# sashajenner/honours

Measured on AMD Instinct MI355X. Metric: raw-signal MB/s (compress+decompress), higher is better.
Workload: dtype u16

## Files before the change

honours_amd/csrc/press_abi.hip:

```cpp

#include <dlfcn.h>
#include <stdarg.h>
#include <stdio.h>
#include <stdlib.h>
#include <string.h>

#include <mutex>
#include <thread>
#include <algorithm>
#include <vector>

#include "../../include/press_hip.h"
#include "press_internal.h"
#include "zs_table.h"

using namespace ph;


static thread_local char g_err[256] = "";

static int fail(int code, const char *fmt, ...)
{
	va_list ap;
	va_start(ap, fmt);
// ... 13 lines not shown

int ph::set_error(int code, const char *fmt, ...)
{
	va_list ap;
	va_start(ap, fmt);
	vsnprintf(g_err, sizeof g_err, fmt, ap);
	va_end(ap);
	return code;
}


namespace {

struct DevBuf;
DevBuf *g_bufs = nullptr;

struct DevBuf {
	void *p = nullptr;
	size_t cap = 0;
	DevBuf *next;
	DevBuf() : next(g_bufs) { g_bufs = this; }
	DevBuf(const DevBuf &) = delete;
	DevBuf &operator=(const DevBuf &) = delete;
	int reserve(size_t n)
	{
		if (n <= cap)
			return 0;
		if (p)
			(void) hipFree(p);
		p = nullptr;
		cap = 0;
		size_t want = n + n / 8 + 4096;
		hipError_t e = hipMalloc(&p, want);
		if (e != hipSuccess)
			return fail(PRESS_HIP_EHIP, "hipMalloc(%zu): %s", want, hipGetErrorString(e));
		cap = want;
		return 0;
	}
	void release()
	{
		if (p)
			(void) hipFree(p);
		p = nullptr;
		cap = 0;
	}
};

struct Ctx {
	bool ready = false;
	int device = -1;
	hipStream_t own = nullptr;
	hipStream_t user = nullptr;
	bool use_user = false;
	DevBuf meta, ex_pos, ex_val, low, huff, chunks, gran, ctl, first_chunk, htiles, hunit, hrec, hlist, hread, hwave, hbits, hend, hmin, cbits;
	DevBuf ztmp, zoff, zoff4, zlen, zhist, ztab, zfirst, zblk, zsbits, zbpos, zbflag, zkcnt, zrd, znb, zn, zdcopy, zdhuf, zdunit, zdtree, zdlong, zdctl, zdseq, zdxblk;
	DevBuf sig, off, nsamp, arena, arena_off, lens, lens2, outn, dense, dense_off;
	uint64_t zs_total = 0;
	uint32_t zs_nhost = 0;
	uint32_t *zs_pin = nullptr;
	hipEvent_t zs_ev = nullptr;
	bool have_table = false;
	bool table_trie = false;
	uint32_t tlen[256];
	uint64_t tbits[256];

	hipStream_t stream() const { return use_user ? user : own; }
};

Ctx g;
std::recursive_mutex g_mu;
#define API_LOCK std::lock_guard<std::recursive_mutex> api_lock_(g_mu)
void staging_release();

int ctx_init()
{
	if (g.ready) {
		HIPCHK(hipSetDevice(g.device));
		return 0;
	}
	int ndev = 0;
	hipError_t e = hipGetDeviceCount(&ndev);
	if (e != hipSuccess || ndev == 0)
		return fail(PRESS_HIP_EHIP, "no HIP device: %s", hipGetErrorString(e));
	if (g.device < 0)
		HIPCHK(hipGetDevice(&g.device));
	HIPCHK(hipSetDevice(g.device));
	HIPCHK(hipStreamCreateWithFlags(&g.own, hipStreamNonBlocking));
	g.ready = true;
	return 0;
}

struct Zstd {
	bool tried = false;
	size_t (*compress)(void *, size_t, const void *, size_t, int) = nullptr;
	size_t (*decompress)(void *, size_t, const void *, size_t) = nullptr;
	size_t (*bound)(size_t) = nullptr;
	unsigned (*is_error)(size_t) = nullptr;
} zstd_fn;

bool zstd_open()
{
	if (zstd_fn.tried)
		return zstd_fn.compress != nullptr;
	zstd_fn.tried = true;
	struct { const char *name; int flags; } names[] = {
		{ "libzstd.so.1", RTLD_NOW | RTLD_LOCAL | RTLD_NOLOAD },
		{ "libzstd.so.1", RTLD_NOW | RTLD_LOCAL },
// ... 296 lines not shown
{
	if (g.meta.reserve(((size_t) nreads + 1) * sizeof(ReadMeta)))
		return PRESS_HIP_EHIP;
	if (is_zs(method)) {
		const int rc = reserve_scratch(zs_inner(method), total_samples, nreads, decode);
		if (rc)
			return rc;
	}
	if (is_zs(method) && decode) {
		ZsBufs z;
		zs_bufs(z, total_samples, nreads, method);
		const size_t nr = (size_t) nreads + 1;
		if (g.ztmp.reserve(2 * zs_tmp_bytes(method, total_samples, nreads)) || g.zoff.reserve(nr * 8) || g.zoff4.reserve(nr * 8) ||
		    g.zlen.reserve(nr * 8) || g.zrd.reserve(nr * sizeof(ZsRead)) || g.zn.reserve(nr * 4) ||
		    g.zdseq.reserve((size_t) z.cap_seq * sizeof(ZsSeq)) || g.zdxblk.reserve((size_t) z.cap_xblk * sizeof(ZsXBlk)) ||
		    g.zdcopy.reserve((size_t) z.cap_copy * sizeof(ZsCopy)) || g.zdhuf.reserve((size_t) z.cap_units * 8 * sizeof(ZsHuf)) ||
		    g.zdunit.reserve((size_t) z.cap_units * sizeof(ZsUnit)) || g.zdtree.reserve((size_t) z.cap_trees * sizeof(ZsTree)) || g.zdlong.reserve((size_t) z.cap_long * sizeof(ZsLong)) ||
		    g.zdctl.reserve(sizeof(ZsDCtl)))
			return PRESS_HIP_EHIP;
	}
	if (is_zs(method) && !decode) {
		const size_t mc = max_chunks_of(total_samples, nreads), mb = max_zblocks_of(total_samples, nreads);
		const size_t nr = (size_t) nreads + 1;
		if (g.ztmp.reserve(zs_tmp_bytes(method, total_samples, nreads)) || g.zoff.reserve(nr * 8) || g.zoff4.reserve(nr * 8) ||
		    g.zlen.reserve(nr * 8) || g.zhist.reserve(nr * 1024) || g.ztab.reserve(nr * sizeof(zs::Table)) ||
		    g.zfirst.reserve(nr * 4) || g.zblk.reserve(mb * 4) || g.zsbits.reserve(mb * 16) || g.zbpos.reserve(mb * 4) ||
		    g.zbflag.reserve(mb) || g.zkcnt.reserve(mc * 4) ||
		    g.zrd.reserve(nr * sizeof(ZsRead)) || g.znb.reserve(64) ||
		    g.ex_pos.reserve((total_samples + 64) * 4) || g.ex_val.reserve((total_samples + 64) * 4))
			return PRESS_HIP_EHIP;
	}
	if (is_svb(method) || is_ex(method)) {
		const size_t mc = max_chunks_of(total_samples, nreads);
		if (g.chunks.reserve(mc * sizeof(ChunkDesc)) || g.gran.reserve(2 * mc * sizeof(uint64_t)) ||
		    g.ctl.reserve(2 * sizeof(ChunkCtl)) || g.first_chunk.reserve(((size_t) nreads + 1) * 4))
			return PRESS_HIP_EHIP;
	}
	if (is_ex(method)) {
		if (g.ex_pos.reserve((total_samples + 64) * 4) || g.ex_val.reserve((total_samples + 64) * 4))
			return PRESS_HIP_EHIP;
		if (!decode && is_shuff(method)) {
			const size_t mc = max_chunks_of(total_samples, nreads);
			if (g.cbits.reserve(mc * sizeof(ChunkBits)))
				return PRESS_HIP_EHIP;
		}
		if (is_rc(method) && g.low.reserve(total_samples + 64))
			return PRESS_HIP_EHIP;
		if (decode && is_shuff(method)) {
			const size_t mt = max_htiles_of(total_samples, nreads);
			if (g.low.reserve(total_samples + 64) || g.htiles.reserve(mt * sizeof(HufTile)) ||
			    g.hunit.reserve(mt * (HUF_HT / 64) * sizeof(HufUnit)) || g.hrec.reserve(mt * HUF_HT * 4) ||
			    g.hlist.reserve(hlist_cap_of(mt) * 8) || g.hread.reserve(((size_t) nreads + 1) * 8) ||
			    g.hwave.reserve(mt * (HUF_HT / 64) * 8) || g.hbits.reserve(mt * (HUF_HT / 64) * 8) ||
			    g.hend.reserve(mt * HUF_HT + 64) ||
			    g.hmin.reserve(((size_t) nreads + 1) * 4))
				return PRESS_HIP_EHIP;
		}
	}
	return 0;
}

}


namespace {
constexpr int KT_RING = 128;
struct KTime {
	bool on = false;
	hipEvent_t ev[2][KT_RING][2];
	bool made = false;
	int n[2] = { 0, 0 };
} kt;
}

namespace ph {
static bool kt_muted = false;
void ktime_mute(bool m) { kt_muted = m; }
void ktime_begin(int which, hipStream_t s)
{
	if (kt.on && !kt_muted && kt.n[which] < KT_RING)
		(void) hipEventRecord(kt.ev[which][kt.n[which]][0], s);
}
void ktime_end(int which, hipStream_t s)
{
	if (kt.on && !kt_muted && kt.n[which] < KT_RING) {
		(void) hipEventRecord(kt.ev[which][kt.n[which]][1], s);
		kt.n[which]++;
	}
}
}

extern "C" int press_hip_kernel_timing(int enable)
{
	API_LOCK;
	int rc = ctx_init();
	if (rc)
		return rc;
	if (enable && !kt.made) {
		for (int w = 0; w < 2; w++)
			for (int i = 0; i < KT_RING; i++)
				for (int e = 0; e < 2; e++)
					HIPCHK(hipEventCreate(&kt.ev[w][i][e]));
		kt.made = true;
	}
	kt.on = enable != 0;
	kt.n[0] = kt.n[1] = 0;
	return 0;
// ... 677 lines not shown
		return rc;
	launch_symbol_counts((const int16_t *) g.sig.p, (const uint64_t *) g.off.p, (const uint32_t *) g.nsamp.p, nreads,
			     (uint64_t *) g.lens.p, g.chunks.p, nchunks, mc, (uint32_t) std::min<uint64_t>(grid, nch), s);
	hipError_t e = hipGetLastError();
	if (e != hipSuccess)
		return fail(PRESS_HIP_EHIP, "kernel launch: %s", hipGetErrorString(e));
	HIPCHK(hipMemcpyAsync(counts, g.lens.p, 257 * 8, hipMemcpyDeviceToHost, s));
	HIPCHK(hipStreamSynchronize(s));
	return 0;
}

extern "C" int press_hip_depress_batch(int method, const uint8_t *in, const uint64_t *in_off,
				       const uint64_t *in_len, uint32_t nreads, int16_t *sig,
				       const uint64_t *off, const uint32_t *n, uint64_t total_samples,
				       uint32_t *out_n, int device_resident)
{
	API_LOCK;
	int rc = ctx_init();
	if (rc)
		return rc;
	if ((rc = check_method(method)))
		return rc;
	if (nreads == 0)
		return 0;
	if (!in || !in_off || !in_len || !sig || !off || !n || !out_n)
		return fail(PRESS_HIP_EARG, "NULL argument");
	hipStream_t s = g.stream();
	if ((rc = reserve_scratch(method, total_samples, nreads, true)))
		return rc;
	g.zs_total = total_samples;

	DecodeArgs a;
	memset(&a, 0, sizeof a);
	a.nreads = nreads;
	a.meta = (ReadMeta *) g.meta.p;
	a.ex_pos = (uint32_t *) g.ex_pos.p;
	a.ex_val = (uint32_t *) g.ex_val.p;
	a.low = (uint8_t *) g.low.p;
	a.huff = (const HuffDev *) g.huff.p;
	a.chunks = (ChunkDesc *) g.chunks.p;
	a.gran = (uint64_t *) g.gran.p;
	a.ctl = (ChunkCtl *) g.ctl.p;
	a.first_chunk = (uint32_t *) g.first_chunk.p;
	a.max_chunks = max_chunks_of(total_samples, nreads);
	if (is_shuff(method)) {
		a.htiles = (HufTile *) g.htiles.p;
		a.hunit = (HufUnit *) g.hunit.p;
		a.hrec = (uint32_t *) g.hrec.p;
		a.hlist = (uint32_t *) g.hlist.p;
		a.hread = (uint32_t *) g.hread.p;
		a.hwave = (uint2 *) g.hwave.p;
		a.hbits = (unsigned long long *) g.hbits.p;
		a.hend = (uint8_t *) g.hend.p;
		a.hmin = (uint32_t *) g.hmin.p;
		a.max_htiles = max_htiles_of(total_samples, nreads);
		a.hlist_cap = (uint32_t) hlist_cap_of(a.max_htiles);
		a.huf_minlen = table_minlen() | (g.table_trie ? HUF_NEEDS_TRIE : 0u);
	}

	if (device_resident) {
		if ((uintptr_t) sig & 15)
			return fail(PRESS_HIP_EARG, "sig must be 16-byte aligned");
		a.in = in;
		a.in_off = in_off;
		a.in_len = in_len;
		a.sig = sig;
		a.off = off;
		a.nsamp = n;
		a.out_n = out_n;
		return launch_depress(method, a, s);
	}

	uint64_t dense = 0;
	std::vector<uint64_t> doff(nreads);
	std::vector<Piece> pc;
	pc.reserve(nreads);
	for (uint32_t r = 0; r < nreads; r++) {
		if (off[r] & 7)
			return fail(PRESS_HIP_EARG, "off[%u] is not a multiple of 8 samples", r);
		if (off[r] + n[r] > total_samples)
			return fail(PRESS_HIP_EARG, "slot %u ends beyond total_samples", r);
		doff[r] = dense;
		if (in_len[r])
			pc.push_back({ const_cast<uint8_t *>(in) + in_off[r], dense, in_len[r] });
		dense += in_len[r];
	}
	if (g.sig.reserve(total_samples * 2 + 64) || g.off.reserve((size_t) nreads * 8) ||
	    g.nsamp.reserve((size_t) nreads * 4) || g.arena.reserve(dense + 64) || g.arena_off.reserve((size_t) nreads * 8) ||
	    g.lens2.reserve((size_t) nreads * 8) || g.outn.reserve((size_t) nreads * 4))
		return PRESS_HIP_EHIP;
	HIPCHK(hipMemcpyAsync(g.arena_off.p, doff.data(), (size_t) nreads * 8, hipMemcpyHostToDevice, s));
	HIPCHK(hipMemcpyAsync(g.lens2.p, in_len, (size_t) nreads * 8, hipMemcpyHostToDevice, s));
	HIPCHK(hipMemcpyAsync(g.off.p, off, (size_t) nreads * 8, hipMemcpyHostToDevice, s));
	HIPCHK(hipMemcpyAsync(g.nsamp.p, n, (size_t) nreads * 4, hipMemcpyHostToDevice, s));
	if (nreads <= 4) {
		for (const Piece &q : pc)
			HIPCHK(hipMemcpyAsync((uint8_t *) g.arena.p + q.dense, q.host, q.len, hipMemcpyHostToDevice, s));
	} else if ((rc = staged_pieces<true>((uint8_t *) g.arena.p, dense, pc, s))) {
		return rc;
	}
	a.in = (const uint8_t *) g.arena.p;
	a.in_off = (const uint64_t *) g.arena_off.p;
	a.in_len = (const uint64_t *) g.lens2.p;
	a.sig = (int16_t *) g.sig.p;
	a.off = (const uint64_t *) g.off.p;
	a.nsamp = (const uint32_t *) g.nsamp.p;
// ... 576 lines not shown
```

honours_amd/csrc/press_huffman.hip:

```cpp

#include "press_internal.h"
#include "press_packed.h"
#include <cstddef>
#include <type_traits>

namespace ph {

#ifdef HUF_STAMPS
__device__ unsigned long long g_hstamp[32];
#define HSTAMP_DECL                                             \
	unsigned long long hs_t = __builtin_amdgcn_s_memtime(); \
	unsigned long long hs_acc[8] = { 0, 0, 0, 0, 0, 0, 0, 0 }
#define HSTAMP(i)                                                              \
	do {     \
		__builtin_amdgcn_sched_barrier(0);                             \
		const unsigned long long hs_n = __builtin_amdgcn_s_memtime(); \
		hs_acc[(i) & 7] += hs_n - hs_t;                                \
		hs_t = hs_n;                                                   \
		__builtin_amdgcn_sched_barrier(0);                             \
	} while (0)
#define HSTAMP_FLUSH(base)                                                     \
	do {                                                                   \
		if ((threadIdx.x & 63) == 0)                                   \
			for (int hs_i = 0; hs_i < 8; hs_i++)                   \
// ... 85 lines not shown
#pragma unroll
		for (int j = 0; j < NDW / 4; j++)
			t[j] = ld16_pay(q + 16 * j);
#pragma unroll
		for (int j = 0; j < NDW % 4; j++)
			x[j] = ld4_pay(q + 4 * (NDW / 4 * 4 + j));
#pragma unroll
		for (int j = 0; j < NDW / 4; j++) {
			col[(4 * j + 0) * S] = t[j].x;
			col[(4 * j + 1) * S] = t[j].y;
			col[(4 * j + 2) * S] = t[j].z;
			col[(4 * j + 3) * S] = t[j].w;
		}
#pragma unroll
		for (int j = 0; j < NDW % 4; j++)
			col[(NDW / 4 * 4 + j) * S] = x[j];
	} else if (nby > lo) {
		uint8_t b[4 * NDW];
#pragma unroll
		for (int i = 0; i < 4 * NDW; i++) {
			const int32_t r = rb0 + i;
			b[i] = src[r < lo ? lo : (r >= nby ? nby - 1 : r)];
		}
#pragma unroll
		for (int j = 0; j < NDW; j++) {
			uint32_t x = 0;
#pragma unroll
			for (int i = 0; i < 4; i++) {
				const int32_t r = rb0 + 4 * j + i;
				x |= (r >= lo && r < nby) ? (uint32_t) b[4 * j + i] << (8 * i) : 0u;
			}
			col[j * S] = x;
		}
	} else {
#pragma unroll
		for (int j = 0; j < NDW; j++)
			col[j * S] = 0;
	}
}

__device__ __forceinline__ int32_t unzz8(uint32_t z) { return (int32_t) (z >> 1) ^ -(int32_t) (z & 1u); }

typedef __attribute__((address_space(3))) const uint32_t *lds_cu32p;
typedef __attribute__((address_space(3))) const uint16_t *lds_cu16p;
typedef __attribute__((address_space(3))) const uint8_t *lds_cu8p;
typedef __attribute__((address_space(3))) uint8_t *lds_u8p;

struct LenTabs {
	alignas(16) uint32_t alut[1 << HUF_LUT_BITS];
	alignas(16) uint16_t flut[1 << HUF_LUT_BITS];
	alignas(16) uint16_t l2ld[HUF_L2_ENTRIES];
};

template <bool TRIE, int S = 64>
__device__ __forceinline__ uint32_t len_scan(const uint32_t *col_, const LenTabs *tabs, const HuffDev *hd, uint32_t start,
					     uint32_t lim, uint32_t nb, uint32_t &cnt, uint32_t &dsum)
{
	const lds_cu32p col = (lds_cu32p) col_;
	const lds_cu32p alut = (lds_cu32p) tabs->alut;
	const lds_cu16p flut = (lds_cu16p) tabs->flut;
	const lds_cu16p l2ld = (lds_cu16p) tabs->l2ld;
	bool bad = start == HEND;
	uint32_t L = lim < nb ? lim : nb;
	if (bad)
		L = 0;
	auto long_ld = [&](uint32_t e, uint32_t wnd) -> uint32_t {
		if (TRIE && e == 0xFFFFFFFFu) {
			const uint32_t t = trie_code(hd, wnd);
			return t ? (((t >> 24) & 31u) | (((uint32_t) unzz8(t & 0xFFu) & 0xFFu) << 8)) : 0u;
		}
		const uint32_t v = l2ld[(e & 0xFFFu) + ((wnd >> HUF_LUT_BITS) & ((1u << ((e >> 12) & 15u)) - 1u))];
		return v == 0xFFFFu ? 0u : v;
	};
	constexpr uint32_t PB = 30;
	const lds_cu32p colm = col - S;
	uint32_t A = (bad ? 0u : start) + PB;
	{
		int32_t LmP = (int32_t) L - HUF_LUT_BITS + (int32_t) PB;
		uint32_t jj = (A >> 5) & 15u;
		uint32_t w0 = colm[__umul24(jj, (uint32_t) S)], w1 = colm[__umul24(jj, (uint32_t) S) + S];
		while ((int32_t) (A & 0x1FFu) <= LmP) {
			const uint32_t pp = A & 0x1FFu;
			{
				const uint32_t w2 = colm[__umul24(jj, (uint32_t) S) + 2 * S];
				const uint32_t wnd = __builtin_amdgcn_alignbit(w1, w0, A);
				const uint32_t e = *(lds_cu32p) ((lds_cu8p) alut + (wnd & (((1u << HUF_LUT_BITS) - 1u) << 2)));
				uint32_t inc = e;
				if ((int32_t) e < 0) {
					const uint32_t ld = long_ld(e, wnd >> 2);
					const uint32_t tot = ld & 0xFFu;
					inc = tot | (1u << HUF_A_CNT) | (((uint32_t) (int32_t) (int8_t) (ld >> 8) & 0x7FFFu) << HUF_A_SUM);
					if (tot - 1u >= L + PB - pp) {
						inc = 0;
						LmP = -1;
					}
				}
				A += inc;
				const uint32_t jn = (A >> 5) & 15u;
				if (jn != jj) {
					w0 = w1;
					w1 = w2;
				}
				jj = jn;
			}
		}
	}
	uint32_t p = (A & 0x1FFu) - PB;
	uint32_t c = (A >> HUF_A_CNT) & 0x7Fu;
	int32_t d = (int32_t) (A << 1) >> 17;
	for (;;) {
		const bool act = p < L;
		if (!any64(act))
			break;
		const uint32_t pp = act ? p : 0u;
		const uint32_t j = pp >> 5;
		const int r0 = (int) __umul24(j, (uint32_t) S);
		const uint32_t wnd = __builtin_amdgcn_alignbit(col[r0 + S], col[r0], pp);
		const uint32_t e = alut[wnd & ((1u << HUF_LUT_BITS) - 1u)];
		const uint32_t f = flut[wnd & ((1u << HUF_LUT_BITS) - 1u)];
		uint32_t tot = e & 15u, n = (e >> HUF_A_CNT) & 15u, len1 = f & 0xFFu;
		int32_t dall = (int32_t) (e << 1) >> 17, d1 = (int32_t) (int8_t) (f >> 8);
		bool fail = false;
		if (any64(act && (int32_t) e < 0)) {
			if (act && (int32_t) e < 0) {
				const uint32_t ld = long_ld(e, wnd);
				tot = len1 = ld & 0xFFu;
				dall = d1 = (int32_t) (int8_t) (ld >> 8);
				fail = tot == 0;
				n = 1;
			}
		}
		const bool fits = pp + tot <= L;
		const bool cut = !fits && pp + len1 > nb;
		if (act && !fail && !cut) {
			p += fits ? tot : len1;
			c += fits ? n : 1u;
			d += fits ? dall : d1;
		}
		if (act && (fail || cut)) {
			bad = true;
			L = 0;
		}
	}
	cnt = c;
	dsum = (uint32_t) d & 0xFFFFu;
	return bad ? HEND : (p >= nb && p < lim ? HEND : p);
}

__device__ __forceinline__ void wave_lds_sync()
{
	__builtin_amdgcn_fence(__ATOMIC_RELEASE, "wavefront");
	__builtin_amdgcn_wave_barrier();
	__builtin_amdgcn_fence(__ATOMIC_ACQUIRE, "wavefront");
}



#ifndef HUF_SYNC_PER_CU
#define HUF_SYNC_PER_CU 2
// ... 69 lines not shown
	__syncthreads();
	uint32_t *img = imgs[threadIdx.x >> 6];
	for (uint32_t i = lane; i < 2 * S; i += 64)
		img[NDW * S + i] = 0;
	uint32_t *col = img + lane;
	HSTAMP_DECL;
	for (;;) {
		uint32_t u = 0;
		if (lane == 0) {
			const uint32_t t = atomicAdd(&s_ticket, 1u);
			const uint32_t c = t / SYNC_UC, slot = t % SYNC_UC;
			unsigned long long *cs = &s_chunk[c & 63u];
			if (slot == 0) {
				u = atomicAdd(&a.ctl->sunits, SYNC_UC);
				__hip_atomic_store(cs, ((unsigned long long) c << 32) | u, __ATOMIC_RELAXED, __HIP_MEMORY_SCOPE_WORKGROUP);
			} else {
				unsigned long long v;
				do {
					v = __hip_atomic_load(cs, __ATOMIC_RELAXED, __HIP_MEMORY_SCOPE_WORKGROUP);
				} while ((uint32_t) (v >> 32) != c);
				u = (uint32_t) v + slot;
			}
		}
		u = uniform(u);
		if (u >= nunits)
			break;
		HSTAMP(0);
		const uint32_t k = u / (HT / 64);
		const uint32_t tid = (u % (HT / 64)) * 64 + lane;
		const HufTile *dp = a.htiles + k;
		const uint32_t nbits_t = uniform(dp->nbits);
		const uint32_t t = uniform(dp->t_last) & 0x7FFFFFFFu;
		const uint8_t *src = a.in + dp->src;
		const int32_t nby = (int32_t) ((nbits_t + 7) >> 3);
		const bool exact = t == 0 && tid < 64;

		wave_lds_sync();
		col_load<NDW, S>(col, src, (int32_t) tid * (OWN / 8), 0, nby);
		wave_lds_sync();
		HSTAMP(1);
		const uint32_t nb = clamp_nb((int64_t) nbits_t - (int64_t) tid * OWN);

		uint32_t f, c0, c, dz, dv;
		{
			const uint32_t g = len_scan<TRIE, S>(col, &lds.tabs, a.huff, (uint32_t) (OWN - RUNUP), OWN, nb, c0, dz);
			const uint32_t gl = (uint32_t) __shfl_up((int) g, 1, 64);
			f = gl == HEND ? HEND : gl - OWN;
			if (gl == HEND && nb > 0)
				f = 0;
			if (lane == 0)
				f = nb > 0 ? 0u : HEND;
		}
		HSTAMP(2);
		const uint32_t e = len_scan<TRIE, S>(col, &lds.tabs, a.huff, f, OWN, nb, c, dv);
		HSTAMP(3);
		const uint32_t e8 = e == HEND ? R_END : e - OWN;
		const uint32_t cw = wave_scan(c), dw = wave_scan(dv);
		const uint32_t f8 = f == HEND ? R_END : f;
		const uint32_t pe8 = (uint32_t) __shfl_up((int) e8, 1, 64);
		const bool broken = lane ? f8 != pe8 : !exact;
		const unsigned long long bm = __ballot(broken);
		a.hrec[(uint64_t) k * HT + tid] = pack_rec(f, c, dv);
		a.hend[(uint64_t) k * HT + tid] = (uint8_t) e8;
		if (lane == 63) {
			a.hwave[u] = make_uint2(cw, dw & 0xFFFFu);
			a.hbits[u] = bm;
		}
		HSTAMP(4);
	}
	HSTAMP_FLUSH(0);
}

constexpr int LIST_WG = 1024;
__global__ __launch_bounds__(LIST_WG) void k_huf_list(DecodeArgs a)
{
	__shared__ uint32_t s_w[LIST_WG / 64];
	__shared__ uint32_t s_base;
	const uint32_t n = min(uniform(a.ctl->nchunks), a.max_htiles) * (HT / 64);
	const uint32_t u = blockIdx.x * LIST_WG + threadIdx.x;
	const uint32_t lane = threadIdx.x & 63, w = threadIdx.x >> 6;
	unsigned long long bm = u < n ? a.hbits[u] : 0ull;
	const uint32_t cnt = (uint32_t) __popcll(bm);
	const uint32_t inc = wave_scan(cnt);
	if (lane == 63)
		s_w[w] = inc;
	__syncthreads();
	uint32_t before = 0, total = 0;
#pragma unroll
	for (int i = 0; i < LIST_WG / 64; i++) {
		const uint32_t x = s_w[i];
		if (i < (int) w)
			before += x;
		total += x;
	}
	if (threadIdx.x == 0)
		s_base = total ? atomicAdd(&a.ctl->ticket2, total) : 0u;
	__syncthreads();
	uint32_t at = s_base + before + inc - cnt;
	while (bm) {
		const uint32_t b = (uint32_t) __builtin_ctzll(bm);
		bm &= bm - 1;
		if (at < a.hlist_cap)
			a.hlist[at] = u * 64 + b;
		at++;
	}
}

#ifndef HUF_FIX_WG
#define HUF_FIX_WG 1024
#endif
constexpr int FIX_WG = HUF_FIX_WG;
template <int RU, bool TRIE>
__global__ __launch_bounds__(FIX_WG) void k_huf_fix(DecodeArgs a, int round, int last)
{
	constexpr int OWN = HufGeo<RU>::OWN, NDW = HufGeo<RU>::NDW, NCOL = HufGeo<RU>::NCOL;
	struct Lds {
		LenTabs tabs;
		uint32_t imgs[FIX_WG / 64][NCOL * 64 + 64];
	};
	__shared__ __attribute__((aligned(16))) Lds lds;
	auto &imgs = lds.imgs;

	const uint32_t *in_list = a.hlist + (round & 1 ? a.hlist_cap : 0u);
	uint32_t *out_list = a.hlist + (round & 1 ? 0u : a.hlist_cap);
	const uint32_t *in_cnt = round ? &a.ctl->lists[round - 1] : &a.ctl->ticket2;
	uint32_t *out_cnt = &a.ctl->lists[round];
	const uint32_t n = min(uniform(*in_cnt), a.hlist_cap);
	if ((uint32_t) FIX_WG * blockIdx.x >= n)
		return;
	const uint32_t lane = threadIdx.x & 63;
	load_len_tables(a.huff, &lds.tabs, FIX_WG);
	__syncthreads();
	uint32_t *col = imgs[threadIdx.x >> 6] + lane;
	for (uint32_t i0 = FIX_WG * blockIdx.x + (threadIdx.x & ~63u); i0 < n; i0 += (uint32_t) FIX_WG * gridDim.x) {
		uint32_t ent = i0 + lane < n ? in_list[i0 + lane] : LIST_NONE;
		if (ent != LIST_NONE && (a.hrec[ent] & 0xFFu) == a.hend[ent - 1])
			ent = LIST_NONE;
		const bool mine = ent != LIST_NONE;
		const uint64_t g = mine ? ent : 1u;
		const uint32_t k = (uint32_t) (g / HT), tid = (uint32_t) (g % HT);
		const HufTile *dp = a.htiles + k;
		const uint32_t nbits_t = mine ? dp->nbits : 0u;
		wave_lds_sync();
		if (mine)
			col_load<NDW>(col, a.in + dp->src, (int32_t) tid * (OWN / 8), 0, (int32_t) ((nbits_t + 7) >> 3));
		wave_lds_sync();
		const uint32_t pe = mine ? a.hend[g - 1] : R_END;
		const uint32_t old_e = mine ? a.hend[g] : R_END;
		uint32_t c2, d2;
		const uint32_t e2 = len_scan<TRIE>(col, &lds.tabs, a.huff, (!mine || pe == R_END) ? HEND : pe, OWN,
					     clamp_nb((int64_t) nbits_t - (int64_t) tid * OWN), c2, d2);
		const uint32_t e8 = e2 == HEND ? R_END : e2 - OWN;
		bool next = false;
		if (mine) {
			const uint32_t old = a.hrec[g];
			a.hrec[g] = pack_rec(pe == R_END ? HEND : pe, c2, d2);
			const long long dc = (long long) (int32_t) (c2 - ((old >> 8) & 0xFFu));
			const unsigned long long dd = (d2 - (old >> 16)) & 0xFFFFu;
			if (dc != 0 || dd != 0)
				atomicAdd(reinterpret_cast<unsigned long long *>(a.hwave + (uint64_t) k * (HT / 64) + (tid >> 6)),
					  (dd << 32) + (unsigned long long) dc);
			if (e8 != old_e) {
				a.hend[g] = (uint8_t) e8;
				const bool more = tid + 1 < HT || !(dp->t_last >> 31);
				next = more && (uint64_t) tid * OWN + OWN < nbits_t;
			}
		}
		list_push(out_list, out_cnt, a.hlist_cap, next, (uint32_t) g + 1, lane);
		if (last && next)
			atomicMin(&a.hmin[dp->read], (uint32_t) g + 1);
	}
}

template <int RU, bool TRIE>
__global__ __launch_bounds__(64) void k_huf_serial(DecodeArgs a)
{
	constexpr int OWN = HufGeo<RU>::OWN, NDW = HufGeo<RU>::NDW, NCOL = HufGeo<RU>::NCOL;
	struct Lds {
		LenTabs tabs;
		uint32_t img[NCOL * 64 + 64];
	};
	__shared__ __attribute__((aligned(16))) Lds lds;
	auto &img = lds.img;

	const uint32_t r = blockIdx.x;
	const uint32_t g0 = uniform(a.hmin[r]);
	if (g0 == 0xFFFFFFFFu)
		return;
	const uint32_t lane = threadIdx.x;
	const uint32_t k0 = uniform(a.hread[2 * r]), nt = uniform(a.hread[2 * r + 1]);
	load_len_tables(a.huff, &lds.tabs, 64);
	uint32_t *col = img + lane;
	const uint64_t gend = (uint64_t) (k0 + nt) * HT;
	for (uint64_t g = g0; g < gend; g++) {
		const uint32_t k = (uint32_t) (g / HT), tid = (uint32_t) (g % HT);
		const HufTile *dp = a.htiles + k;
		const uint32_t nbits_t = uniform(dp->nbits);
		if ((uint64_t) tid * OWN >= nbits_t)
			break;
		const uint32_t pe = uniform((uint32_t) __hip_atomic_load(a.hend + g - 1, __ATOMIC_RELAXED, __HIP_MEMORY_SCOPE_AGENT));
		const uint32_t rec = uniform(__hip_atomic_load(a.hrec + g, __ATOMIC_RELAXED, __HIP_MEMORY_SCOPE_AGENT));
		if ((rec & 0xFFu) == pe)
			continue;
		wave_lds_sync();
		if (lane == 0)
			col_load<NDW>(col, a.in + dp->src, (int32_t) tid * (OWN / 8), 0, (int32_t) ((nbits_t + 7) >> 3));
		wave_lds_sync();
		uint32_t c2, d2;
		const uint32_t e2 = len_scan<TRIE>(col, &lds.tabs, a.huff, (lane || pe == R_END) ? HEND : pe, OWN,
					     clamp_nb((int64_t) nbits_t - (int64_t) tid * OWN), c2, d2);
		if (lane == 0) {
			a.hrec[g] = pack_rec(pe == R_END ? HEND : pe, c2, d2);
			atomicAdd(reinterpret_cast<unsigned long long *>(a.hwave + (uint64_t) k * (HT / 64) + (tid >> 6)),
				  ((unsigned long long) ((d2 - (rec >> 16)) & 0xFFFFu) << 32) +
					  (unsigned long long) (long long) (int32_t) (c2 - ((rec >> 8) & 0xFFu)));
			__hip_atomic_store(a.hend + g, (uint8_t) (e2 == HEND ? R_END : e2 - OWN), __ATOMIC_RELAXED, __HIP_MEMORY_SCOPE_AGENT);
		}
		__builtin_amdgcn_fence(__ATOMIC_RELEASE, "agent");
	}
}

__device__ __forceinline__ uint32_t unzz16(uint32_t z) { return ((z >> 1) ^ (0u - (z & 1u))) & 0xFFFFu; }

__device__ __forceinline__ void keys_below2(const uint32_t *pos, uint32_t nex, uint32_t ka, uint32_t kb, uint32_t &ea, uint32_t &eb)
{
	uint32_t la = 0, lb = 0;
	for (uint32_t step = nex ? 1u << (31 - __builtin_clz(nex)) : 0u; step; step >>= 1) {
		const uint32_t ia = la + step - 1, ib = lb + step - 1;
		const uint32_t pa = ia < nex ? pos[ia] : 0u, pb = ib < nex ? pos[ib] : 0u;
		if (ia < nex && pa - ia < ka)
			la += step;
		if (ib < nex && pb - ib < kb)
			lb += step;
	}
	ea = la;
	eb = lb;
}

template <int RU>
__global__ __launch_bounds__(HT) void k_huf_chain(DecodeArgs a)
{
	constexpr uint32_t UB = 64 * HufGeo<RU>::OWN / 8;
	constexpr uint32_t UPT = HT / 64;
	__shared__ uint32_t s_w[HT / 64], s_wd[HT / 64];
	__shared__ unsigned long long s_cum;

	const uint32_t r = blockIdx.x;
	const uint32_t tid = threadIdx.x;
	const uint32_t k0 = uniform(a.hread[2 * r]), nt = uniform(a.hread[2 * r + 1]);
	if (!nt)
		return;
	const uint32_t nu = nt * UPT;
	const uint2 *hw = a.hwave + (uint64_t) k0 * UPT;
	if (tid == 0)
		s_cum = 0;
	__syncthreads();
	{
		uint64_t c = 0;
		for (uint32_t u = tid; u < nu; u += HT)
			c += hw[u].x;
		if (c)
			atomicAdd(&s_cum, (unsigned long long) c);
	}
	const uint32_t want = uniform(a.htiles[k0].want);
	const uint32_t nex = uniform(a.meta[r].nex);
// ... 50 lines not shown
#pragma unroll
		for (int w2 = 0; w2 < HT / 64; w2++) {
			const uint32_t x = s_w[w2], y = s_wd[w2];
			if (w2 < (int) (tid >> 6)) {
				before += x;
				dbefore += y;
			}
			total += x;
			dtotal += y;
		}
		if (u < nu) {
			const uint64_t ob = cum + before + inc - c;
			const uint32_t L0 = ob > 0xFFFFFFFFull ? 0xFFFFFFFFu : (uint32_t) ob;
			const uint32_t quota = L0 >= want ? 0u : (c < want - L0 ? c : want - L0);
			const uint32_t L1 = L0 + quota;
			uint32_t Ea = 0, Eb = 0;
			if (fused && quota) {
				keys_below2(pos, nex, L0, L1, Ea, Eb);
				if (L1 == nlow)
					Eb = nex;
			}
			uint32_t bz = zd0;
			if (L0) {
				bz = unzz16(zd0) + ((dcum + dbefore + dinc - dt) & 0xFFFFu);
				if (Ea) {
					const uint32_t pv = val[Ea - 1];
					bz += (pv >> 16) + unzz16(pv & 0xFFFFu);
				}
				bz &= 0xFFFFu;
			}
			const uint64_t src = src0 + (uint64_t) u * UB;
			const int64_t nby = nby0 - (int64_t) u * UB;
			const uint32_t nbyc = nby <= 0 ? 0u : (nby > (int64_t) HUF_U_NBY ? HUF_U_NBY : (uint32_t) nby);
			uint4 *d = reinterpret_cast<uint4 *>(a.hunit + (uint64_t) k0 * UPT + u);
			d[0] = make_uint4((uint32_t) src, (uint32_t) (src >> 32) | (bz << 16), (uint32_t) o0, (uint32_t) (o0 >> 32));
			d[1] = make_uint4(L0, quota | (nbyc << 14) | ((q & 15u) << 26) | (fused ? 1u << 30 : 0u), Ea, Eb - Ea);
		}
		cum += total;
		dcum += dtotal;
		__syncthreads();
	}
	static_assert(HUF_U_QUOTA >= 64u * 255u, "a unit's quota");
	if (tid == 0) {
		a.meta[r].nlow = nlow;
		if (fused)
			a.hread[2 * r + 1] = nt | HUF_FUSED;
	}
}


constexpr uint32_t EMIT_STG = 4096;

template <bool TRIE>
__device__ __forceinline__ void emit_codes(const uint32_t *col_, const uint32_t *lut_, const uint16_t *lut2_,
					   const HuffDev *hd, uint32_t p, uint32_t nmine, uint8_t *wp_)
{
	const lds_cu32p col = (lds_cu32p) col_;
	const lds_cu8p lut = (lds_cu8p) lut_;
	const lds_cu16p lut2 = (lds_cu16p) lut2_;
	auto long_entry = [&](uint32_t e, uint32_t wnd) -> uint32_t {
		if (TRIE && e == 0xFFFFFFFFu) {
			const uint32_t t = trie_code(hd, wnd);
			return t ? ((t & 0xFFFFFF00u) | ((uint32_t) unzz8(t & 0xFFu) & 0xFFu)) : 0u;
		}
		const uint32_t e2 = lut2[(e & 0xFFFu) + ((wnd >> HUF_LUT_BITS) & ((1u << ((e >> 12) & 15u)) - 1u))];
		return e2 == 0xFFFFu ? 0u : (((uint32_t) unzz8(e2 & 0xFFu) & 0xFFu) | (e2 & 0x1F00u) | ((e2 & 0x1F00u) << 16));
	};
	typedef lds_u8p WP;
	WP w = (WP) wp_;
	const WP wend = w + nmine;
	WP wlim = nmine ? wend - 1 : w;
	constexpr uint32_t PB = 30;
	const lds_cu32p colm = col - 64;
	uint32_t pp = p + PB;
	uint32_t jj = pp >> 5;
	uint32_t w0 = colm[__umul24(jj, 64u)], w1 = colm[__umul24(jj, 64u) + 64];
	while (w < wlim) {
		{
			const uint32_t w2 = colm[__umul24(jj, 64u) + 128];
			const uint32_t wnd = __builtin_amdgcn_alignbit(w1, w0, pp);
			uint32_t e = *(lds_cu32p) (lut + (wnd & (((1u << HUF_LUT_BITS) - 1u) << 2)));
			if (e >= HUF_LONG)
				e = long_entry(e, wnd >> 2);
			w[0] = (uint8_t) e;
			w[1] = (uint8_t) (e >> 16);
			w += 1u + ((e >> 29) & 1u);
			pp += (e >> 8) & 0x1Fu;
			const uint32_t jn = pp >> 5;
			if (jn != jj) {
				w0 = w1;
				w1 = w2;
			}
			jj = jn;
		}
	}
	if (w < wend) {
		const uint32_t wnd = __builtin_amdgcn_alignbit(w1, w0, pp);
		uint32_t e = *(lds_cu32p) (lut + (wnd & (((1u << HUF_LUT_BITS) - 1u) << 2)));
		if (e >= HUF_LONG)
			e = long_entry(e, wnd >> 2);
		w[0] = (uint8_t) e;
	}
}


__device__ __forceinline__ uint32_t lower_bound_u32(const uint32_t *p, uint32_t n, uint32_t key)
{
	uint32_t lo = 0, hi = n;
	while (lo < hi) {
		const uint32_t mid = (lo + hi) >> 1;
		if (p[mid] < key)
			lo = mid + 1;
		else
			hi = mid;
	}
	return lo;
}

template <typename LOWAT>
__device__ __forceinline__ void gather8(LOWAT lowat, const uint32_t *pos, const uint32_t *val, uint32_t zd0,
					uint32_t i0, uint32_t Ia, uint32_t Ib, uint32_t e_first, uint32_t e_cnt,
					uint32_t v[4])
{
	v[0] = v[1] = v[2] = v[3] = 0;
	const uint32_t lo = i0 > Ia ? i0 : Ia;
	const uint32_t hi = i0 + 8 < Ib ? i0 + 8 : Ib;
	if (lo >= hi)
		return;
	const uint32_t uf = lo ? lo - 1 : 0;
	const uint32_t e_end = e_first + e_cnt;
	uint32_t e = e_first + lower_bound_u32(pos + e_first, e_cnt, uf);
	uint32_t l = uf - e;
	uint32_t nextpos = e < e_end ? pos[e] : 0xFFFFFFFFu;
#pragma unroll
	for (int h = 0; h < 8; h++) {
		const uint32_t i = i0 + h;
		if (i >= lo && i < hi) {
			uint32_t dl;
			if (i == 0) {
				dl = unzz16(zd0);
			} else if (i - 1 == nextpos) {
				dl = unzz16(val[e] & 0xFFFFu);
				e++;
				nextpos = e < e_end ? pos[e] : 0xFFFFFFFFu;
			} else {
				dl = lowat(l) & 0xFFFFu;
				l++;
			}
			v[h >> 1] |= dl << (16 * (h & 1));
		}
	}
}

struct EmitRead {
// ... 174 lines not shown
	uint32_t *col = img[wv] + lane;
	uint8_t *stg = stg_all.s[wv];
	__syncthreads();
	auto draw = [&]() -> uint32_t {
		uint32_t u = 0;
		if (lane == 0) {
			const uint32_t t = atomicAdd(&s_ticket, 1u);
			const uint32_t c = t / EMIT_UC, slot = t % EMIT_UC;
			unsigned long long *cs = &s_chunk[c & 63u];
			if (slot == 0) {
				u = atomicAdd(&a.ctl->units, EMIT_UC);
				__hip_atomic_store(cs, ((unsigned long long) c << 32) | u, __ATOMIC_RELAXED, __HIP_MEMORY_SCOPE_WORKGROUP);
			} else {
				unsigned long long v;
				do {
					v = __hip_atomic_load(cs, __ATOMIC_RELAXED, __HIP_MEMORY_SCOPE_WORKGROUP);
				} while ((uint32_t) (v >> 32) != c);
				u = (uint32_t) v + slot;
			}
		}
		return uniform(u);
	};
	static_assert(offsetof(HufUnit, obase) == 16 && offsetof(HufUnit, ecnt) == 28, "the plan is read as eight dwords");
	static_assert(63 * (OWN / 8) + 4 * NDW <= HUF_U_NBY, "HufUnit::qnf's byte count tells whether every lane's bytes lie inside");
	auto fetch_unit = [&](uint32_t u) -> uint32_t {
		uint32_t v = 0;
		if (u < nunits && lane < 8)
			v = reinterpret_cast<const uint32_t *>(a.hunit + u)[lane];
		return v;
	};
	struct Unit {
		uint32_t u, obase, quota, nby, fused, q, bz, ea, ecnt;
		uint64_t srco, roff;
	};
	auto resolve = [&](uint32_t u, uint32_t tv) -> Unit {
		auto at = [&](int i) -> uint32_t { return (uint32_t) __builtin_amdgcn_readlane((int) tv, i); };
		Unit U;
		U.u = u;
		const uint32_t hb = at(1), qnf = at(5);
		U.srco = ((uint64_t) (hb & 0xFFFFu) << 32) | at(0);
		U.bz = hb >> 16;
		U.roff = ((uint64_t) at(3) << 32) | at(2);
		U.obase = at(4);
		U.quota = qnf & HUF_U_QUOTA;
		U.nby = (qnf >> 14) & HUF_U_NBY;
		U.q = (qnf >> 26) & 15u;
		U.fused = qnf >> 30;
		U.ea = at(6);
		U.ecnt = at(7);
		return U;
	};
	struct Stage2 {
		uint32_t pay[NDW];
		uint32_t rec, pe;
		bool fast;
	};
	auto issue2 = [&](const Unit &U, Stage2 &S) {
		const int32_t rb0 = (int32_t) lane * (OWN / 8);
		S.fast = U.nby >= 63 * (OWN / 8) + 4 * NDW;
		const uint8_t *q = a.in + U.srco + rb0;
		if (S.fast) {
			uint4 t[NDW / 4 ? NDW / 4 : 1];
#pragma unroll
			for (int j = 0; j < NDW / 4; j++)
				t[j] = ld16_pay(q + 16 * j);
#pragma unroll
			for (int j = 0; j < NDW % 4; j++)
				S.pay[NDW / 4 * 4 + j] = ld4_pay(q + 4 * (NDW / 4 * 4 + j));
#pragma unroll
			for (int j = 0; j < NDW / 4; j++) {
				S.pay[4 * j + 0] = t[j].x;
				S.pay[4 * j + 1] = t[j].y;
				S.pay[4 * j + 2] = t[j].z;
				S.pay[4 * j + 3] = t[j].w;
			}
		}
		S.rec = a.hrec[(uint64_t) U.u * 64 + lane];
		S.pe = (U.ecnt <= 64 && lane < U.ecnt) ? a.ex_pos[U.roff + U.ea + lane] : 0xFFFFFFFFu;
	};
	auto land2 = [&](const Unit &U, const Stage2 &S) {
		wave_lds_sync();
		if (S.fast) {
#pragma unroll
			for (int j = 0; j < NDW; j++)
				col[j * 64] = S.pay[j];
		} else {
			col_load<NDW>(col, a.in + U.srco, (int32_t) lane * (OWN / 8), 0, (int32_t) U.nby);
		}
		wave_lds_sync();
	};
	HSTAMP_DECL;
	const uint32_t u_first = draw();
	if (u_first >= nunits)
		return;
	Unit U = resolve(u_first, fetch_unit(u_first)), Un = {}, Unn = {};
	Stage2 S, Sn = {};
	issue2(U, S);
	land2(U, S);
	uint32_t u_nxt = draw();
	if (u_nxt < nunits)
		Un = resolve(u_nxt, fetch_unit(u_nxt));
	for (;;) {
		const uint32_t u_nn = draw();
		const uint32_t tv_nn = fetch_unit(u_nn);
		const bool more = u_nxt < nunits;
		if (more)
			issue2(Un, Sn);
		HSTAMP(0);
		const uint32_t rec = S.rec;
		const uint32_t quota = U.quota;
		const uint32_t obase = U.obase;
		const uint64_t roff = U.roff;
		const uint32_t cnt = (rec >> 8) & 0xFFu;
		const uint32_t inc = wave_scan(cnt);
		const bool fused = U.fused != 0;
		const uint32_t ex = inc - cnt;
		const uint32_t f = rec & 0xFFu;
		const uint32_t p0 = f == R_END ? 0u : f;
		uint32_t nmine = (ex >= quota || f == R_END) ? 0u : (cnt < quota - ex ? cnt : quota - ex);
		nmine = ex >= EMIT_STG ? 0u : (nmine < EMIT_STG - ex ? nmine : EMIT_STG - ex);
		HSTAMP(2);
		{
#if defined(EMIT_ABL) && EMIT_ABL == 3
			if (a.nreads == 0x7FFFFFFFu)
#endif
			emit_codes<TRIE>(col, lut, lut2, a.huff, p0, nmine, stg + ex);
			HSTAMP(3);
			const uint32_t pe = S.pe;
			if (more)
				land2(Un, Sn);
			else
				wave_lds_sync();
			if (u_nn < nunits)
				Unn = resolve(u_nn, tv_nn);
			HSTAMP(1);
			if (fused) {
				if (quota) {
					EmitRead R;
					R.pos = a.ex_pos + roff;
					R.val = a.ex_val + roff;
					R.out = a.sig + roff;
					R.zd0 = U.bz;
					R.q = U.q;
					EmitPlan P;
					P.L0 = obase;
					P.L1 = obase + quota;
					P.Ea = U.ea;
					P.ecnt = U.ecnt;
					P.Ia = obase ? obase + U.ea + 1 : 0u;
					P.Ib = P.L1 + U.ea + U.ecnt + 1;
					P.base = obase ? U.bz : 0u;
					P.pe = pe;
					HSTAMP(4);
#if defined(EMIT_ABL) && EMIT_ABL == 2
					if (a.nreads == 0x7FFFFFFFu)
#endif
					emit_samples16(stg, R, P, lane);
					HSTAMP(5);
				}
			} else {
				uint8_t *dst = a.low + roff + obase;
				for (uint32_t o = lane * 16; o < quota; o += 64 * 16) {
					uint4 v = *reinterpret_cast<const uint4 *>(stg + o);
					v = make_uint4(zz_bytes(v.x), zz_bytes(v.y), zz_bytes(v.z), zz_bytes(v.w));
					if (o + 16 <= quota) {
						__builtin_memcpy(dst + o, &v, 16);
					} else {
						const uint32_t vv[4] = { v.x, v.y, v.z, v.w };
						for (uint32_t b = 0; o + b < quota; b++)
							dst[o + b] = (uint8_t) (vv[b >> 2] >> (8 * (b & 3)));
					}
				}
			}
			wave_lds_sync();
		}
		HSTAMP(6);
		if (!more)
			break;
		U = Un;
// ... 140 lines not shown
```

honours_amd/csrc/press_internal.h:

```cpp
#pragma once

#include <hip/hip_runtime.h>
#include <stdint.h>

namespace ph {

enum ExFmt : int {
	EXF_VBE21 = 0,
	EXF_VBBE21 = 1,
	EXF_VBSBE21 = 2,
	EXF_VBSSE21 = 3,
	EXF_EXZD = 4
};

struct ReadMeta {
	uint32_t nex;
	uint32_t ored;
	uint32_t zd0;
	uint32_t q;
	uint32_t hdr;
	uint32_t seclen;
	uint32_t nlow;
	uint32_t status;
};

constexpr int HUF_LUT_BITS = 12;
constexpr int HUF_L2_ENTRIES = 3072;
constexpr int HUF_L2_IDS = 64;
struct HuffDev {
	uint32_t enc[256];
	uint16_t lut[1 << HUF_LUT_BITS];
	int16_t child[1024][2];
	int16_t leaf[1024];
	uint32_t minlen, maxlen;
	uint16_t lut2[HUF_L2_ENTRIES];
	uint16_t l2off[256];
	uint8_t l2bits[256];
	alignas(16) uint32_t lut32[1 << HUF_LUT_BITS];
	alignas(16) uint32_t mlut[1 << HUF_LUT_BITS];
	alignas(16) uint16_t l2ld[HUF_L2_ENTRIES];
	alignas(16) uint32_t alut[1 << HUF_LUT_BITS];
	alignas(16) uint16_t flut[1 << HUF_LUT_BITS];
};
constexpr uint32_t HUF_A_CNT = 9, HUF_A_SUM = 16;
constexpr uint32_t HUF_NEEDS_TRIE = 0x80000000u;
constexpr uint32_t HUF_L2_NONE = HUF_L2_ENTRIES - 1;
constexpr uint32_t HUF_MLONG = 1u << 31;
constexpr uint32_t HUF_M_MAXN = 8;
constexpr uint32_t HUF_LONG = 1u << 30;
constexpr uint32_t HUF_TWO = 1u << 29;

constexpr int HUF_HT = 256;
struct HufUnit {
	uint32_t src_lo;
	uint32_t src_hi_bz;
	uint64_t roff;
	uint32_t obase;
	uint32_t qnf;
	uint32_t ea, ecnt;
};
static_assert(sizeof(HufUnit) == 32, "HufUnit");
constexpr uint32_t HUF_U_QUOTA = 0x3FFFu, HUF_U_NBY = 0xFFFu;
constexpr uint32_t HUF_FUSED = 0x80000000u;

constexpr uint32_t CHUNK = 32768;
struct ChunkDesc {
	uint64_t sig_off;
	uint64_t out_base;
	uint32_t n;
	uint32_t j;
	uint32_t read;
	uint32_t cap_ok;
	uint64_t ebefore;
	uint32_t ecnt[4];
	uint16_t kmask[4];
};
static_assert(sizeof(ChunkDesc) == 64, "ChunkDesc is one 64-byte line");
struct ChunkBits {
	uint64_t before;
	uint32_t q[4];
	uint32_t pad[2];
};
struct ChunkCtl {
	uint32_t ticket;
	uint32_t pad0[31];
	uint32_t nchunks;
	uint32_t pad1[31];
	uint32_t ticket2;
	uint32_t pad2[31];
	uint32_t lists[32];
	uint32_t units;
	uint32_t pad4[31];
	uint32_t sunits;
	uint32_t pad5[31];
};

struct BatchArgs {
	const int16_t *sig;
	const uint64_t *off;
	const uint32_t *nsamp;
	uint8_t *out;
	const uint64_t *out_off;
	uint64_t *out_len;
	ReadMeta *meta;
	uint32_t *ex_pos;
	uint32_t *ex_val;
	const HuffDev *huff;
	uint32_t nreads;
	ChunkDesc *chunks;
	uint64_t *gran;
	ChunkCtl *ctl;
	uint32_t max_chunks;
	ChunkBits *cbits;
	uint8_t *low_tmp;
	uint32_t *first_chunk;
	uint32_t *zhist;
	uint32_t *zkcnt;
};

struct HufTile {
	uint64_t src;
	uint64_t low;
	uint32_t nbits;
	uint32_t t_last;
	uint32_t read;
	uint32_t want;
};

struct DecodeArgs {
	const uint8_t *in;
	const uint64_t *in_off;
	const uint64_t *in_len;
	int16_t *sig;
	const uint64_t *off;
	const uint32_t *nsamp;
	uint32_t *out_n;
	ReadMeta *meta;
	uint32_t *ex_pos;
	uint32_t *ex_val;
	uint8_t *low;
	const HuffDev *huff;
	uint32_t nreads;
	ChunkDesc *chunks;
	uint64_t *gran;
	ChunkCtl *ctl;
	uint32_t *first_chunk;
	uint32_t max_chunks;
	HufTile *htiles;
	HufUnit *hunit;
	uint32_t *hrec;
	uint32_t *hlist;
	uint8_t *hend;
	uint32_t *hmin;
	uint32_t *hread;
	uint2 *hwave;
	unsigned long long *hbits;
	uint32_t max_htiles;
	uint32_t hlist_cap;
	uint32_t huf_minlen;
};

struct ZsRead {
	uint32_t nk, nd;
	uint32_t knz;
	uint32_t mode;
	uint32_t dbase;
	uint32_t plen;
	uint32_t pad[2];
};
struct ZsCopy {
	uint64_t src, dst;
	uint32_t n, fill;
};
struct ZsHuf {
	uint64_t src, dst;
	uint32_t cs, R;
	uint32_t four;
	uint32_t pad;
};
struct ZsUnit {
	uint32_t read, tree, count, pad;
};
struct ZsLong {
	ZsHuf h;
	uint32_t tree, read, pad[2];
};
struct ZsTree {
	uint8_t w[256];
	uint32_t tl, pad[3];
};
struct ZsSeq {
	uint32_t ll, ml, off;
};
struct ZsXBlk {
	uint64_t lit;
	uint64_t dst;
	uint32_t seq0, nseq;
	uint32_t tail;
	uint32_t next;
};
struct ZsDCtl {
	uint32_t ncopy, pad0[1023];
	uint32_t nunits, pad1[1023];
	uint32_t ntrees, pad2[1023];
	uint32_t nseq, pad3[1023];
// ... 63 lines not shown
```

Measured before the change: 764,600.

## Split Huffman emit into two interleaved decode streams using recorded midpoints

The length-scan pass now also records, per lane, a midpoint bit position and symbol count, stored in a new hmid buffer. The emit stage then decodes two independent halves of each lane's segment in one interleaved loop, raising instruction-level parallelism on the serial LUT lookup chain. In exchange it adds extra global writes and reads for hmid, more registers, and dummy stores to a junk row when one stream finishes early.

Result: slower. 750,100, median of 2 (-1.9%).

```diff
diff --git a/honours_amd/csrc/press_abi.hip b/honours_amd/csrc/press_abi.hip
--- a/honours_amd/csrc/press_abi.hip
+++ b/honours_amd/csrc/press_abi.hip
@@ -89,7 +89,7 @@
 	hipStream_t own = nullptr;
 	hipStream_t user = nullptr;
 	bool use_user = false;
-	DevBuf meta, ex_pos, ex_val, low, huff, chunks, gran, ctl, first_chunk, htiles, hunit, hrec, hlist, hread, hwave, hbits, hend, hmin, cbits;
+	DevBuf meta, ex_pos, ex_val, low, huff, chunks, gran, ctl, first_chunk, htiles, hunit, hrec, hlist, hread, hwave, hbits, hend, hmid, hmin, cbits;
 	DevBuf ztmp, zoff, zoff4, zlen, zhist, ztab, zfirst, zblk, zsbits, zbpos, zbflag, zkcnt, zrd, znb, zn, zdcopy, zdhuf, zdunit, zdtree, zdlong, zdctl, zdseq, zdxblk;
 	DevBuf sig, off, nsamp, arena, arena_off, lens, lens2, outn, dense, dense_off;
 	uint64_t zs_total = 0;
@@ -492,7 +492,7 @@
 			    g.hunit.reserve(mt * (HUF_HT / 64) * sizeof(HufUnit)) || g.hrec.reserve(mt * HUF_HT * 4) ||
 			    g.hlist.reserve(hlist_cap_of(mt) * 8) || g.hread.reserve(((size_t) nreads + 1) * 8) ||
 			    g.hwave.reserve(mt * (HUF_HT / 64) * 8) || g.hbits.reserve(mt * (HUF_HT / 64) * 8) ||
-			    g.hend.reserve(mt * HUF_HT + 64) ||
+			    g.hend.reserve(mt * HUF_HT + 64) || g.hmid.reserve(mt * HUF_HT * 2) ||
 			    g.hmin.reserve(((size_t) nreads + 1) * 4))
 				return PRESS_HIP_EHIP;
 		}
@@ -1276,6 +1276,8 @@
 		a.hwave = (uint2 *) g.hwave.p;
 		a.hbits = (unsigned long long *) g.hbits.p;
 		a.hend = (uint8_t *) g.hend.p;
+		a.hmid = (uint16_t *) g.hmid.p;
+		a.hmid = (uint16_t *) g.hmid.p;
 		a.hmin = (uint32_t *) g.hmin.p;
 		a.max_htiles = max_htiles_of(total_samples, nreads);
 		a.hlist_cap = (uint32_t) hlist_cap_of(a.max_htiles);
diff --git a/honours_amd/csrc/press_huffman.hip b/honours_amd/csrc/press_huffman.hip
--- a/honours_amd/csrc/press_huffman.hip
+++ b/honours_amd/csrc/press_huffman.hip
@@ -161,9 +161,9 @@
 	alignas(16) uint16_t l2ld[HUF_L2_ENTRIES];
 };
 
-template <bool TRIE, int S = 64>
+template <bool TRIE, int S = 64, uint32_t MP = 0>
 __device__ __forceinline__ uint32_t len_scan(const uint32_t *col_, const LenTabs *tabs, const HuffDev *hd, uint32_t start,
-					     uint32_t lim, uint32_t nb, uint32_t &cnt, uint32_t &dsum)
+					     uint32_t lim, uint32_t nb, uint32_t &cnt, uint32_t &dsum, uint32_t *mid = nullptr)
 {
 	const lds_cu32p col = (lds_cu32p) col_;
 	const lds_cu32p alut = (lds_cu32p) tabs->alut;
@@ -184,6 +184,7 @@
 	constexpr uint32_t PB = 30;
 	const lds_cu32p colm = col - S;
 	uint32_t A = (bad ? 0u : start) + PB;
+	uint32_t M = 0;
 	{
 		int32_t LmP = (int32_t) L - HUF_LUT_BITS + (int32_t) PB;
 		uint32_t jj = (A >> 5) & 15u;
@@ -205,6 +206,8 @@
 					}
 				}
 				A += inc;
+				if (MP)
+					M = pp < MP + PB ? A : M;
 				const uint32_t jn = (A >> 5) & 15u;
 				if (jn != jj) {
 					w0 = w1;
@@ -214,6 +217,8 @@
 			}
 		}
 	}
+	if (MP)
+		*mid = (M & 0x1FFu) >= MP + PB ? ((M & 0x1FFu) - PB) | (((M >> HUF_A_CNT) & 0x7Fu) << 8) : HUF_NO_MID;
 	uint32_t p = (A & 0x1FFu) - PB;
 	uint32_t c = (A >> HUF_A_CNT) & 0x7Fu;
 	int32_t d = (int32_t) (A << 1) >> 17;
@@ -389,7 +394,8 @@
 				f = nb > 0 ? 0u : HEND;
 		}
 		HSTAMP(2);
-		const uint32_t e = len_scan<TRIE, S>(col, &lds.tabs, a.huff, f, OWN, nb, c, dv);
+		uint32_t mid;
+		const uint32_t e = len_scan<TRIE, S, OWN / 2>(col, &lds.tabs, a.huff, f, OWN, nb, c, dv, &mid);
 		HSTAMP(3);
 		const uint32_t e8 = e == HEND ? R_END : e - OWN;
 		const uint32_t cw = wave_scan(c), dw = wave_scan(dv);
@@ -399,6 +405,7 @@
 		const unsigned long long bm = __ballot(broken);
 		a.hrec[(uint64_t) k * HT + tid] = pack_rec(f, c, dv);
 		a.hend[(uint64_t) k * HT + tid] = (uint8_t) e8;
+		a.hmid[(uint64_t) k * HT + tid] = (uint16_t) mid;
 		if (lane == 63) {
 			a.hwave[u] = make_uint2(cw, dw & 0xFFFFu);
 			a.hbits[u] = bm;
@@ -484,14 +491,15 @@
 		wave_lds_sync();
 		const uint32_t pe = mine ? a.hend[g - 1] : R_END;
 		const uint32_t old_e = mine ? a.hend[g] : R_END;
-		uint32_t c2, d2;
-		const uint32_t e2 = len_scan<TRIE>(col, &lds.tabs, a.huff, (!mine || pe == R_END) ? HEND : pe, OWN,
-					     clamp_nb((int64_t) nbits_t - (int64_t) tid * OWN), c2, d2);
+		uint32_t c2, d2, m2;
+		const uint32_t e2 = len_scan<TRIE, 64, OWN / 2>(col, &lds.tabs, a.huff, (!mine || pe == R_END) ? HEND : pe, OWN,
+							      clamp_nb((int64_t) nbits_t - (int64_t) tid * OWN), c2, d2, &m2);
 		const uint32_t e8 = e2 == HEND ? R_END : e2 - OWN;
 		bool next = false;
 		if (mine) {
 			const uint32_t old = a.hrec[g];
 			a.hrec[g] = pack_rec(pe == R_END ? HEND : pe, c2, d2);
+			a.hmid[g] = (uint16_t) m2;
 			const long long dc = (long long) (int32_t) (c2 - ((old >> 8) & 0xFFu));
 			const unsigned long long dd = (d2 - (old >> 16)) & 0xFFFFu;
 			if (dc != 0 || dd != 0)
@@ -543,11 +551,12 @@
 		if (lane == 0)
 			col_load<NDW>(col, a.in + dp->src, (int32_t) tid * (OWN / 8), 0, (int32_t) ((nbits_t + 7) >> 3));
 		wave_lds_sync();
-		uint32_t c2, d2;
-		const uint32_t e2 = len_scan<TRIE>(col, &lds.tabs, a.huff, (lane || pe == R_END) ? HEND : pe, OWN,
-					     clamp_nb((int64_t) nbits_t - (int64_t) tid * OWN), c2, d2);
+		uint32_t c2, d2, m2;
+		const uint32_t e2 = len_scan<TRIE, 64, OWN / 2>(col, &lds.tabs, a.huff, (lane || pe == R_END) ? HEND : pe, OWN,
+							      clamp_nb((int64_t) nbits_t - (int64_t) tid * OWN), c2, d2, &m2);
 		if (lane == 0) {
 			a.hrec[g] = pack_rec(pe == R_END ? HEND : pe, c2, d2);
+			a.hmid[g] = (uint16_t) m2;
 			atomicAdd(reinterpret_cast<unsigned long long *>(a.hwave + (uint64_t) k * (HT / 64) + (tid >> 6)),
 				  ((unsigned long long) ((d2 - (rec >> 16)) & 0xFFFFu) << 32) +
 					  (unsigned long long) (long long) (int32_t) (c2 - ((rec >> 8) & 0xFFu)));
@@ -704,8 +713,8 @@
 constexpr uint32_t EMIT_STG = 4096;
 
 template <bool TRIE>
-__device__ __forceinline__ void emit_codes(const uint32_t *col_, const uint32_t *lut_, const uint16_t *lut2_,
-					   const HuffDev *hd, uint32_t p, uint32_t nmine, uint8_t *wp_)
+__device__ __forceinline__ void emit_codes(const uint32_t *col_, const uint32_t *lut_, const uint16_t *lut2_, const HuffDev *hd,
+					   uint32_t pa, uint32_t na, uint32_t pb, uint32_t nb, uint8_t *wp_, uint8_t *junk_)
 {
 	const lds_cu32p col = (lds_cu32p) col_;
 	const lds_cu8p lut = (lds_cu8p) lut_;
@@ -718,40 +727,60 @@
 		const uint32_t e2 = lut2[(e & 0xFFFu) + ((wnd >> HUF_LUT_BITS) & ((1u << ((e >> 12) & 15u)) - 1u))];
 		return e2 == 0xFFFFu ? 0u : (((uint32_t) unzz8(e2 & 0xFFu) & 0xFFu) | (e2 & 0x1F00u) | ((e2 & 0x1F00u) << 16));
 	};
+	auto look = [&](uint32_t wnd) -> uint32_t { return *(lds_cu32p) (lut + (wnd & (((1u << HUF_LUT_BITS) - 1u) << 2))); };
 	typedef lds_u8p WP;
-	WP w = (WP) wp_;
-	const WP wend = w + nmine;
-	WP wlim = nmine ? wend - 1 : w;
+	const WP junk = (WP) junk_;
+	WP wa = (WP) wp_, wb = wa + na;
+	const WP wenda = wb, wendb = wb + nb;
+	const WP wlima = na ? wenda - 1 : wa, wlimb = nb ? wendb - 1 : wb;
 	constexpr uint32_t PB = 30;
 	const lds_cu32p colm = col - 64;
-	uint32_t pp = p + PB;
-	uint32_t jj = pp >> 5;
-	uint32_t w0 = colm[__umul24(jj, 64u)], w1 = colm[__umul24(jj, 64u) + 64];
-	while (w < wlim) {
-		{
-			const uint32_t w2 = colm[__umul24(jj, 64u) + 128];
-			const uint32_t wnd = __builtin_amdgcn_alignbit(w1, w0, pp);
-			uint32_t e = *(lds_cu32p) (lut + (wnd & (((1u << HUF_LUT_BITS) - 1u) << 2)));
-			if (e >= HUF_LONG)
-				e = long_entry(e, wnd >> 2);
-			w[0] = (uint8_t) e;
-			w[1] = (uint8_t) (e >> 16);
-			w += 1u + ((e >> 29) & 1u);
-			pp += (e >> 8) & 0x1Fu;
-			const uint32_t jn = pp >> 5;
-			if (jn != jj) {
-				w0 = w1;
-				w1 = w2;
-			}
-			jj = jn;
-		}
-	}
-	if (w < wend) {
-		const uint32_t wnd = __builtin_amdgcn_alignbit(w1, w0, pp);
-		uint32_t e = *(lds_cu32p) (lut + (wnd & (((1u << HUF_LUT_BITS) - 1u) << 2)));
-		if (e >= HUF_LONG)
-			e = long_entry(e, wnd >> 2);
-		w[0] = (uint8_t) e;
+	uint32_t ppa = pa + PB, ppb = pb + PB;
+	uint32_t ja = ppa >> 5, jb = ppb >> 5;
+	uint32_t a0 = colm[__umul24(ja, 64u)], a1 = colm[__umul24(ja, 64u) + 64];
+	uint32_t b0 = colm[__umul24(jb, 64u)], b1 = colm[__umul24(jb, 64u) + 64];
+	bool ga = wa < wlima, gb = wb < wlimb;
+	while (ga || gb) {
+		const uint32_t a2 = colm[__umul24(ja, 64u) + 128], b2 = colm[__umul24(jb, 64u) + 128];
+		const uint32_t wnda = __builtin_amdgcn_alignbit(a1, a0, ppa), wndb = __builtin_amdgcn_alignbit(b1, b0, ppb);
+		uint32_t ea = look(wnda), eb = look(wndb);
+		if (ga && ea >= HUF_LONG)
+			ea = long_entry(ea, wnda >> 2);
+		if (gb && eb >= HUF_LONG)
+			eb = long_entry(eb, wndb >> 2);
+		const WP sa = ga ? wa : junk, sb = gb ? wb : junk;
+		sa[0] = (uint8_t) ea;
+		sa[1] = (uint8_t) (ea >> 16);
+		sb[0] = (uint8_t) eb;
+		sb[1] = (uint8_t) (eb >> 16);
+		wa += ga ? 1u + ((ea >> 29) & 1u) : 0u;
+		wb += gb ? 1u + ((eb >> 29) & 1u) : 0u;
+		ppa += ga ? (ea >> 8) & 0x1Fu : 0u;
+		ppb += gb ? (eb >> 8) & 0x1Fu : 0u;
+		const uint32_t jna = ppa >> 5, jnb = ppb >> 5;
+		if (jna != ja) {
+			a0 = a1;
+			a1 = a2;
+		}
+		if (jnb != jb) {
+			b0 = b1;
+			b1 = b2;
+		}
+		ja = jna;
+		jb = jnb;
+		ga = wa < wlima;
+		gb = wb < wlimb;
+	}
+	const bool ta = wa < wenda, tb = wb < wendb;
+	if (ta || tb) {
+		const uint32_t wnda = __builtin_amdgcn_alignbit(a1, a0, ppa), wndb = __builtin_amdgcn_alignbit(b1, b0, ppb);
+		uint32_t ea = look(wnda), eb = look(wndb);
+		if (ta && ea >= HUF_LONG)
+			ea = long_entry(ea, wnda >> 2);
+		if (tb && eb >= HUF_LONG)
+			eb = long_entry(eb, wndb >> 2);
+		(ta ? wa : junk)[0] = (uint8_t) ea;
+		(tb ? wb : junk)[0] = (uint8_t) eb;
 	}
 }
 
@@ -1032,7 +1061,7 @@
 	};
 	struct Stage2 {
 		uint32_t pay[NDW];
-		uint32_t rec, pe;
+		uint32_t rec, mid, pe;
 		bool fast;
 	};
 	auto issue2 = [&](const Unit &U, Stage2 &S) {
@@ -1056,6 +1085,7 @@
 			}
 		}
 		S.rec = a.hrec[(uint64_t) U.u * 64 + lane];
+		S.mid = a.hmid[(uint64_t) U.u * 64 + lane];
 		S.pe = (U.ecnt <= 64 && lane < U.ecnt) ? a.ex_pos[U.roff + U.ea + lane] : 0xFFFFFFFFu;
 	};
 	auto land2 = [&](const Unit &U, const Stage2 &S) {
@@ -1087,7 +1117,7 @@
 		if (more)
 			issue2(Un, Sn);
 		HSTAMP(0);
-		const uint32_t rec = S.rec;
+		const uint32_t rec = S.rec, mid = S.mid;
 		const uint32_t quota = U.quota;
 		const uint32_t obase = U.obase;
 		const uint64_t roff = U.roff;
@@ -1099,12 +1129,15 @@
 		const uint32_t p0 = f == R_END ? 0u : f;
 		uint32_t nmine = (ex >= quota || f == R_END) ? 0u : (cnt < quota - ex ? cnt : quota - ex);
 		nmine = ex >= EMIT_STG ? 0u : (nmine < EMIT_STG - ex ? nmine : EMIT_STG - ex);
+		const uint32_t cm = mid == HUF_NO_MID ? EMIT_STG : mid >> 8;
+		const uint32_t na = nmine < cm ? nmine : cm;
+		const uint32_t pm = na < nmine ? (mid & 0xFFu) : p0;
 		HSTAMP(2);
 		{
 #if defined(EMIT_ABL) && EMIT_ABL == 3
 			if (a.nreads == 0x7FFFFFFFu)
 #endif
-			emit_codes<TRIE>(col, lut, lut2, a.huff, p0, nmine, stg + ex);
+			emit_codes<TRIE>(col, lut, lut2, a.huff, p0, na, pm, nmine - na, stg + ex, (uint8_t *) pad_row);
 			HSTAMP(3);
 			const uint32_t pe = S.pe;
 			if (more)
diff --git a/honours_amd/csrc/press_internal.h b/honours_amd/csrc/press_internal.h
--- a/honours_amd/csrc/press_internal.h
+++ b/honours_amd/csrc/press_internal.h
@@ -62,6 +62,7 @@
 static_assert(sizeof(HufUnit) == 32, "HufUnit");
 constexpr uint32_t HUF_U_QUOTA = 0x3FFFu, HUF_U_NBY = 0xFFFu;
 constexpr uint32_t HUF_FUSED = 0x80000000u;
+constexpr uint32_t HUF_NO_MID = 0xFFFFu;
 
 constexpr uint32_t CHUNK = 32768;
 struct ChunkDesc {
@@ -151,6 +152,7 @@
 	uint32_t *hrec;
 	uint32_t *hlist;
 	uint8_t *hend;
+	uint16_t *hmid;
 	uint32_t *hmin;
 	uint32_t *hread;
 	uint2 *hwave;
```
